# andrewcsmith/soundsym

Measured on NVIDIA B200. Metric: dtw_cell_updates_per_s, higher is better.
Workload: dtype f16 (packed-half DP scan on f16 tensor-core costs; winners refined in f64)

## Files before the change

soundsym_b200/csrc/dtw_h2.cu:

```cuda
#include <algorithm>
#include <atomic>
#include <type_traits>

#include "match.cuh"
#include "tc_common.cuh"

namespace ss {

int dtw_rescore_finalize(ss_dict* d, ss_queries* q, int k, int kp, uint32_t nslots, const uint32_t* d_slot_qid, double eps,
                         const float* d_max_na, const float* d_max_nb, const float* d_slot_max_na, int bound_mode, uint8_t* d_uncert_flag,
                         uint32_t* d_out_idx, double* d_out_dist);

int dtw_second_chance(ss_dict* d, ss_queries* q, int k, int kp, uint32_t nslots, const uint32_t* d_slot_qid, const unsigned long long* d_partial,
                      uint32_t nlists, const unsigned long long* d_thr, double eps, const float* d_max_na, const float* d_max_nb,
                      const float* d_slot_max_na, int bound_mode, uint8_t* d_uncert_flag, uint32_t* d_out_idx, double* d_out_dist);

constexpr int kH2Slots = 2;
constexpr int kH2SlotCols = 64;
constexpr int kH2DpWarps = 4 * kH2Slots;
constexpr int kH2DpThreads = kH2DpWarps * 32;
constexpr int kH2Threads = (kH2DpWarps + 1) * 32;
constexpr int kH2DescInt4 = 4;
constexpr int kH2In = 1, kH2Out = 2;
constexpr int kH2ARing = 32;
constexpr int kH2MaxLong = 2048;
constexpr int kH2Pipes = 2;
constexpr int kH2PDpWarps = kH2Pipes * kH2DpWarps;
constexpr int kH2PDpThreads = kH2PDpWarps * 32;
constexpr int kH2PThreads = (kH2PDpWarps + 4) * 32;
constexpr int kH2PRegsDp = 112, kH2PRegsProd = 32;
static_assert(kH2PDpThreads * kH2PRegsDp + 128 * kH2PRegsProd == kH2PThreads * 96, "setmaxnreg budget must match the launch pool");

struct H2Params {
    const unsigned char* a_blocks;
    const uint64_t* group_off;
    const uint32_t* group_len;
    const uint32_t* slot_len;
    uint32_t ngroups;
    const unsigned char* tiles;
    const int4* desc;
    const uint32_t* slice_tile;
    uint32_t nslices, slice_begin;
    unsigned long long* partial;
    uint32_t max_len;
    float inv_s;
    unsigned long long* thr;
    float* dbg;
    uint32_t dbg_nseg;
    __half2* bnd;
    uint32_t bnd_rows;
    float eta;
    unsigned long long* timeline;
};
__device__ __forceinline__ unsigned long long h2_now() {
    unsigned long long t;
    asm volatile("mov.u64 %0, %%globaltimer;" : "=l"(t));
    return t;
}

template <int N>
__device__ __forceinline__ void h2_ld(uint32_t taddr, __half2* v);
template <>
__device__ __forceinline__ void h2_ld<4>(uint32_t taddr, __half2* v) {
    uint32_t r[4];
    asm volatile("tcgen05.ld.sync.aligned.32x32b.x4.pack::16b.b32 {%0, %1, %2, %3}, [%4];\n" : "=r"(r[0]), "=r"(r[1]), "=r"(r[2]), "=r"(r[3]) : "r"(taddr));
#pragma unroll
    for (int i = 0; i < 4; i++) v[i] = *reinterpret_cast<__half2*>(&r[i]);
}
template <>
__device__ __forceinline__ void h2_ld<8>(uint32_t taddr, __half2* v) {
    uint32_t r[8];
    asm volatile("tcgen05.ld.sync.aligned.32x32b.x8.pack::16b.b32 {%0, %1, %2, %3, %4, %5, %6, %7}, [%8];\n"
                 : "=r"(r[0]), "=r"(r[1]), "=r"(r[2]), "=r"(r[3]), "=r"(r[4]), "=r"(r[5]), "=r"(r[6]), "=r"(r[7])
                 : "r"(taddr));
#pragma unroll
    for (int i = 0; i < 8; i++) v[i] = *reinterpret_cast<__half2*>(&r[i]);
}
template <>
__device__ __forceinline__ void h2_ld<16>(uint32_t taddr, __half2* v) {
    uint32_t r[16];
    asm volatile(
        "tcgen05.ld.sync.aligned.32x32b.x16.pack::16b.b32 {%0, %1, %2, %3, %4, %5, %6, %7, %8, %9, %10, %11, %12, %13, %14, %15}, [%16];\n"
        : "=r"(r[0]), "=r"(r[1]), "=r"(r[2]), "=r"(r[3]), "=r"(r[4]), "=r"(r[5]), "=r"(r[6]), "=r"(r[7]), "=r"(r[8]), "=r"(r[9]), "=r"(r[10]),
          "=r"(r[11]), "=r"(r[12]), "=r"(r[13]), "=r"(r[14]), "=r"(r[15])
        : "r"(taddr));
#pragma unroll
    for (int i = 0; i < 16; i++) v[i] = *reinterpret_cast<__half2*>(&r[i]);
}
template <int NG>
__device__ __forceinline__ void h2_ld_row(uint32_t taddr, __half2 (&v)[4 * NG]) {
    constexpr int N = 4 * NG;
    int done = 0;
    if constexpr (N >= 32) {
        h2_ld<16>(taddr, v);
        h2_ld<16>(taddr + 32, v + 16);
        done = 32;
    } else if constexpr (N >= 16) {
        h2_ld<16>(taddr, v);
        done = 16;
    }
    if constexpr ((N & 8) != 0) {
        h2_ld<8>(taddr + 2 * done, v + done);
        done += 8;
    }
    if constexpr ((N & 4) != 0) h2_ld<4>(taddr + 2 * done, v + done);
}

__device__ __forceinline__ __half2 h2_min3(__half2 a, __half2 b, __half2 c) { return __hmin2(__hmin2(a, b), c); }
__device__ __forceinline__ __half2 h2_inf() {
    const uint32_t bits = 0x7C007C00u;
    return *reinterpret_cast<const __half2*>(&bits);
}
__device__ __forceinline__ __half2 h2_zero() {
    const uint32_t bits = 0u;
    return *reinterpret_cast<const __half2*>(&bits);
}
__device__ __forceinline__ __half2 h2_combine(__half2 a, __half2 b) {
    const uint32_t r = __byte_perm(*reinterpret_cast<uint32_t*>(&a), *reinterpret_cast<uint32_t*>(&b), 0x7610);
    return *reinterpret_cast<const __half2*>(&r);
}
__device__ __forceinline__ int h2_len_of(const int4& sc, int e) { return (int)((((e < 4) ? (uint32_t)sc.x : (uint32_t)sc.y) >> (8 * (e & 3))) & 0xFFu); }
__device__ __forceinline__ int h2_seg_of(const int4& sa, const int4& sb, int e) {
    return e == 0 ? sa.x : e == 1 ? sa.y : e == 2 ? sa.z : e == 3 ? sa.w : e == 4 ? sb.x : e == 5 ? sb.y : e == 6 ? sb.z : sb.w;
}
__device__ __forceinline__ uint32_t h2_selp(uint32_t a, uint32_t b, int pick_a) {
    uint32_t r;
    asm("{\n.reg .pred q;\nsetp.ne.s32 q, %3, 0;\nselp.b32 %0, %1, %2, q;\n}\n" : "=r"(r) : "r"(a), "r"(b), "r"(pick_a));
    return r;
}
__device__ __forceinline__ __half2 h2_pick4(const __half2* v, int r) {
    const uint32_t v0 = *reinterpret_cast<const uint32_t*>(&v[0]), v1 = *reinterpret_cast<const uint32_t*>(&v[1]);
    const uint32_t v2 = *reinterpret_cast<const uint32_t*>(&v[2]), v3 = *reinterpret_cast<const uint32_t*>(&v[3]);
    const uint32_t lo = h2_selp(v1, v0, r & 1), hi = h2_selp(v3, v2, r & 1);
    const uint32_t o = h2_selp(hi, lo, r & 2);
    return *reinterpret_cast<const __half2*>(&o);
}

template <int NG>
__device__ __forceinline__ void h2_band(const __half2 (&tm0)[4 * NG], const __half2 (&tm1)[4 * NG], __half2 (&d)[4 * NG], __half2 dinit, __half2 (&c0l)[4]) {
    __half2 left0 = h2_inf(), diag0 = dinit, left1 = h2_inf();
#pragma unroll
    for (int j = 0; j < 4 * NG; j++) {
        const __half2 up0 = d[j];
        const __half2 c0 = __hadd2(tm0[j], h2_min3(left0, up0, diag0));
        const __half2 c1 = __hadd2(tm1[j], h2_min3(left1, c0, left0));
        diag0 = up0;
        left0 = c0;
        left1 = c1;
        d[j] = c1;
        if (j >= 4 * (NG - 1)) c0l[j - 4 * (NG - 1)] = c0;
    }
}
template <int NG>
__device__ __forceinline__ void h2_band_io(const __half2 (&tm0)[4 * NG], const __half2 (&tm1)[4 * NG], __half2 (&d)[4 * NG], __half2 l0, __half2 dg0,
                                           __half2 l1, __half2 (&c0l)[4], __half2& o0, __half2& o1) {
    __half2 left0 = l0, diag0 = dg0, left1 = l1;
#pragma unroll
    for (int j = 0; j < 4 * NG; j++) {
        const __half2 up0 = d[j];
        const __half2 c0 = __hadd2(tm0[j], h2_min3(left0, up0, diag0));
        const __half2 c1 = __hadd2(tm1[j], h2_min3(left1, c0, left0));
        diag0 = up0;
        left0 = c0;
        left1 = c1;
        d[j] = c1;
        if (j >= 4 * (NG - 1)) c0l[j - 4 * (NG - 1)] = c0;
    }
    o0 = left0, o1 = left1;
}
template <int NG>
__device__ __forceinline__ void h2_band_row_io(const __half2 (&tm)[4 * NG], __half2 (&d)[4 * NG], __half2 l0, __half2 dg0, __half2& o0) {
    __half2 left = l0, diag = dg0;
#pragma unroll
    for (int j = 0; j < 4 * NG; j++) {
        const __half2 up = d[j];
        const __half2 cur = __hadd2(tm[j], h2_min3(left, up, diag));
        diag = up;
        left = cur;
        d[j] = cur;
    }
    o0 = left;
}
template <int NG>
__device__ __forceinline__ void h2_band_row(const __half2 (&tm)[4 * NG], __half2 (&d)[4 * NG], __half2 dinit) {
    __half2 left = h2_inf(), diag = dinit;
#pragma unroll
    for (int j = 0; j < 4 * NG; j++) {
        const __half2 up = d[j];
        const __half2 cur = __hadd2(tm[j], h2_min3(left, up, diag));
        diag = up;
        left = cur;
        d[j] = cur;
    }
}

template <int NG, int J0, int J1>
__device__ __forceinline__ void h2_band_cols(const __half2* tm0, const __half2* tm1, __half2 (&d)[4 * NG], __half2& left0, __half2& diag0,
                                             __half2& left1, __half2 (&c0l)[4]) {
#pragma unroll
    for (int j = J0; j < J1; j++) {
        const __half2 up0 = d[j];
        const __half2 c0 = __hadd2(tm0[j - J0], h2_min3(left0, up0, diag0));
        const __half2 c1 = __hadd2(tm1[j - J0], h2_min3(left1, c0, left0));
        diag0 = up0;
        left0 = c0;
        left1 = c1;
        d[j] = c1;
        if (j >= 4 * (NG - 1)) c0l[j - 4 * (NG - 1)] = c0;
    }
}

struct H2PipeCursor {
    uint32_t par, full, taddr;
    __device__ __forceinline__ void wait() const {
        mb_wait_addr(full, par);
        tc_fence_after();
    }
    __device__ __forceinline__ void release() {
        tc_fence_before();
        mb_arrive_elect(full + 16);
        par ^= 1u;
    }
};

template <int NB, int NG, class Cur>
__device__ __forceinline__ void h2_step2(Cur& cur, __half2 (&d)[NB][4 * NG], __half2 dinit, __half2 (&c0l)[NB][4]) {
    constexpr int kBandCols = kH2SlotCols / NB;
    cur.wait();
    const uint32_t taddr = cur.taddr;
    if constexpr (std::is_same<Cur, H2PipeCursor>::value && NB == 1) {
        static_assert(NG >= 5, "NB = 1 tiles have 5..8 column groups");
        __half2 left0 = h2_inf(), diag0 = dinit, left1 = h2_inf();
        {
            __half2 a0[16], a1[16];
            h2_ld_row<4>(taddr, a0);
            h2_ld_row<4>(taddr + kTcN, a1);
            tc_wait_ld();
            h2_band_cols<NG, 0, 16>(a0, a1, d[0], left0, diag0, left1, c0l[0]);
        }
        __half2 b0[4 * (NG - 4)], b1[4 * (NG - 4)];
        h2_ld_row<NG - 4>(taddr + 32, b0);
        h2_ld_row<NG - 4>(taddr + kTcN + 32, b1);
        tc_wait_ld();
        cur.release();
        h2_band_cols<NG, 16, 4 * NG>(b0, b1, d[0], left0, diag0, left1, c0l[0]);
    } else if constexpr (std::is_same<Cur, H2PipeCursor>::value) {
        constexpr int H = NB / 2;
        {
            __half2 tm0[H][4 * NG], tm1[H][4 * NG];
#pragma unroll
            for (int b = 0; b < H; b++) {
                h2_ld_row<NG>(taddr + b * kBandCols, tm0[b]);
                h2_ld_row<NG>(taddr + kTcN + b * kBandCols, tm1[b]);
            }
            tc_wait_ld();
#pragma unroll
            for (int b = 0; b < H; b++) h2_band<NG>(tm0[b], tm1[b], d[b], dinit, c0l[b]);
        }
        __half2 tm0[H][4 * NG], tm1[H][4 * NG];
#pragma unroll
        for (int b = 0; b < H; b++) {
            h2_ld_row<NG>(taddr + (H + b) * kBandCols, tm0[b]);
            h2_ld_row<NG>(taddr + kTcN + (H + b) * kBandCols, tm1[b]);
        }
        tc_wait_ld();
        cur.release();
#pragma unroll
        for (int b = 0; b < H; b++) h2_band<NG>(tm0[b], tm1[b], d[H + b], dinit, c0l[H + b]);
    } else {
        __half2 tm0[NB][4 * NG], tm1[NB][4 * NG];
#pragma unroll
        for (int b = 0; b < NB; b++) {
            h2_ld_row<NG>(taddr + b * kBandCols, tm0[b]);
            h2_ld_row<NG>(taddr + kTcN + b * kBandCols, tm1[b]);
        }
        tc_wait_ld();
        cur.release();
#pragma unroll
        for (int b = 0; b < NB; b++) h2_band<NG>(tm0[b], tm1[b], d[b], dinit, c0l[b]);
    }
}

template <int NB, int NG, class Cur>
__device__ __forceinline__ void h2_tile(uint32_t L, uint32_t lmin, uint32_t Lm, const int4& sc, Cur& cur, __half2 (&res)[NB]) {
    __half2 d[NB][4 * NG];
#pragma unroll
    for (int b = 0; b < NB; b++) {
#pragma unroll
        for (int j = 0; j < 4 * NG; j++) d[b][j] = h2_inf();
        res[b] = h2_inf();
    }
    __half2 dinit = h2_zero();
    const uint32_t nfull = L >> 1;
    const uint32_t ncap = min((lmin - 1) >> 1, nfull);
    uint32_t st = 0;
    if constexpr (std::is_same<Cur, H2PipeCursor>::value) {
#pragma unroll 1
        for (; st < ncap; st++) {
            __half2 c0l[NB][4];
            h2_step2<NB, NG>(cur, d, dinit, c0l);
            dinit = h2_inf();
        }
    } else {
        if (st < ncap && cur.buf) {
            __half2 c0l[NB][4];
            h2_step2<NB, NG>(cur, d, dinit, c0l);
            dinit = h2_inf();
            st++;
        }
        if (st + 2 <= ncap) {
            const uint32_t full0 = cur.full, taddr0 = cur.taddr;
            uint32_t par = cur.par;
#pragma unroll 1
            for (; st + 2 <= ncap; st += 2) {
                __half2 c0l[NB][4];
                TcCursor c0 = {0u, par, full0, taddr0, cur.full_sum, cur.taddr_sum};
                h2_step2<NB, NG>(c0, d, dinit, c0l);
                TcCursor c1 = {1u, par, full0 + 8u, taddr0 + (uint32_t)kTcBufCols, cur.full_sum, cur.taddr_sum};
                h2_step2<NB, NG>(c1, d, h2_inf(), c0l);
                dinit = h2_inf();
                par ^= 1u;
            }
            cur.par = par;
        }
        if (st < ncap) {
            __half2 c0l[NB][4];
            h2_step2<NB, NG>(cur, d, dinit, c0l);
            dinit = h2_inf();
            st++;
        }
    }
#pragma unroll 1
    for (; st < nfull; st++) {
        __half2 c0l[NB][4];
        h2_step2<NB, NG>(cur, d, dinit, c0l);
        dinit = h2_inf();
        const bool end0 = 2 * st + 1 == Lm, end1 = 2 * st + 2 == Lm;
#pragma unroll
        for (int b = 0; b < NB; b++) {
            const int ra = (h2_len_of(sc, 2 * b) - 1) & 3, rb = (h2_len_of(sc, 2 * b + 1) - 1) & 3;
            const __half2 e0 = h2_combine(h2_pick4(c0l[b], ra), h2_pick4(c0l[b], rb));
            const __half2 e1 = h2_combine(h2_pick4(&d[b][4 * (NG - 1)], ra), h2_pick4(&d[b][4 * (NG - 1)], rb));
            res[b] = end0 ? e0 : (end1 ? e1 : res[b]);
        }
    }
    if (L & 1) {
        constexpr int kBandCols = kH2SlotCols / NB;
        cur.wait();
        __half2 tm0[NB][4 * NG];
#pragma unroll
        for (int b = 0; b < NB; b++) h2_ld_row<NG>(cur.taddr + b * kBandCols, tm0[b]);
        tc_wait_ld();
        cur.release();
#pragma unroll
        for (int b = 0; b < NB; b++) {
            h2_band_row<NG>(tm0[b], d[b], dinit);
            const int ra = (h2_len_of(sc, 2 * b) - 1) & 3, rb = (h2_len_of(sc, 2 * b + 1) - 1) & 3;
            const __half2 e = h2_combine(h2_pick4(&d[b][4 * (NG - 1)], ra), h2_pick4(&d[b][4 * (NG - 1)], rb));
            res[b] = (L == Lm) ? e : res[b];
        }
    }
}

template <int NG, bool IN, bool OUT>
__device__ __forceinline__ void h2_tile_strip(uint32_t L, uint32_t lmin, uint32_t Lm, const int4& sc, TcCursor& cur, __half2* bnd, __half2& res) {
    constexpr uint32_t kStride = kH2DpThreads;
    __half2 d[4 * NG];
#pragma unroll
    for (int j = 0; j < 4 * NG; j++) d[j] = h2_inf();
    res = h2_inf();
    __half2 prev_b = IN ? h2_inf() : h2_zero();
    const uint32_t nfull = L >> 1;
    const uint32_t ncap = OUT ? nfull : min((lmin - 1) >> 1, nfull);
    const int ra = (h2_len_of(sc, 0) - 1) & 3, rb = (h2_len_of(sc, 1) - 1) & 3;
#pragma unroll 1
    for (uint32_t st = 0; st < nfull; st++) {
        __half2 b0 = h2_inf(), b1 = h2_inf();
        if (IN) b0 = bnd[(size_t)(2 * st) * kStride], b1 = bnd[(size_t)(2 * st + 1) * kStride];
        cur.wait();
        const uint32_t taddr = cur.taddr;
        __half2 tm0[4 * NG], tm1[4 * NG], c0l[4], o0, o1;
        h2_ld_row<NG>(taddr, tm0);
        h2_ld_row<NG>(taddr + kTcN, tm1);
        tc_wait_ld();
        cur.release();
        h2_band_io<NG>(tm0, tm1, d, b0, prev_b, b1, c0l, o0, o1);
        prev_b = IN ? b1 : h2_inf();
        if (OUT) {
            bnd[(size_t)(2 * st) * kStride] = o0;
            bnd[(size_t)(2 * st + 1) * kStride] = o1;
        } else if (st >= ncap) {
            const bool end0 = 2 * st + 1 == Lm, end1 = 2 * st + 2 == Lm;
            const __half2 e0 = h2_combine(h2_pick4(c0l, ra), h2_pick4(c0l, rb));
            const __half2 e1 = h2_combine(h2_pick4(&d[4 * (NG - 1)], ra), h2_pick4(&d[4 * (NG - 1)], rb));
            res = end0 ? e0 : (end1 ? e1 : res);
        }
    }
    if (L & 1) {
        __half2 b0 = h2_inf();
        if (IN) b0 = bnd[(size_t)(L - 1) * kStride];
        cur.wait();
        __half2 tm0[4 * NG], o0;
        h2_ld_row<NG>(cur.taddr, tm0);
        tc_wait_ld();
        cur.release();
        h2_band_row_io<NG>(tm0, d, b0, prev_b, o0);
        if (OUT) {
            bnd[(size_t)(L - 1) * kStride] = o0;
        } else {
            const __half2 e = h2_combine(h2_pick4(&d[4 * (NG - 1)], ra), h2_pick4(&d[4 * (NG - 1)], rb));
            res = (L == Lm) ? e : res;
        }
    }
}

template <int KP, int NB, bool DBG = false>
__global__ void __launch_bounds__(kH2Threads, 1) k_dtw_scan_h2(const H2Params p) {
    extern __shared__ unsigned char smem_raw[];
    unsigned char* smem = smem_raw + ((128u - (s32(smem_raw) & 127u)) & 127u);
    unsigned char* sA = smem;
    unsigned char* sB = smem + (size_t)p.max_len * kTcATileBytes;
    uint64_t* bars = reinterpret_cast<uint64_t*>(sB + kTcStages * kTcBTileBytes);
    uint64_t* a_full = bars;
    uint64_t* b_full = bars + 1;
    uint64_t* b_empty = b_full + kTcStages;
    uint64_t* t_full = bars + 10;
    uint64_t* t_empty = bars + 12;
    uint32_t* tmem_slot = reinterpret_cast<uint32_t*>(bars + 14);
    unsigned long long* topk = reinterpret_cast<unsigned long long*>(bars + 32);

    const int warp = threadIdx.x >> 5, lane = threadIdx.x & 31;
    uint32_t g, slice;
    if (blockIdx.x < p.ngroups) {
        g = blockIdx.x, slice = p.slice_begin;
    } else {
        const uint32_t r = blockIdx.x - p.ngroups;
        g = r / (p.nslices - 1), slice = p.slice_begin + 1 + r % (p.nslices - 1);
    }
    asm volatile("griddepcontrol.launch_dependents;" ::: "memory");
    const uint32_t glen = p.group_len[g];
    const uint32_t L = glen & 0xFFFFu, lmin = glen >> 16;
    const uint32_t t0 = p.slice_tile[slice], t1 = p.slice_tile[slice + 1];
    const uint32_t ntiles = t1 - t0;
    unsigned long long* tl = p.timeline ? p.timeline + ((size_t)(p.slice_begin * p.ngroups) + blockIdx.x) * 8 : nullptr;
    if (tl && threadIdx.x == 0) {
        unsigned smid;
        asm("mov.u32 %0, %%smid;" : "=r"(smid));
        tl[0] = h2_now(), tl[4] = smid | ((unsigned long long)NB << 16) | ((unsigned long long)g << 32), tl[7] = ((unsigned long long)L << 32) | ntiles;
    }

    if (threadIdx.x == 0) {
        mb_init(a_full, 1);
        for (int s = 0; s < kTcStages; s++) mb_init(&b_full[s], 1), mb_init(&b_empty[s], 1);
        for (int s = 0; s < 2; s++) mb_init(&t_full[s], 1), mb_init(&t_empty[s], kH2DpWarps);
        asm volatile("fence.mbarrier_init.release.cluster;" ::: "memory");
    }
    if (warp == kH2DpWarps) {
        asm volatile("tcgen05.alloc.cta_group::1.sync.aligned.shared::cta.b32 [%0], %1;" ::"r"(s32(tmem_slot)), "r"(512u) : "memory");
        asm volatile("tcgen05.relinquish_alloc_permit.cta_group::1.sync.aligned;" ::: "memory");
    }
    tc_fence_before();
    __syncthreads();
    tc_fence_after();
    const uint32_t tmem_base = *tmem_slot;
    if (tl && threadIdx.x == 0) tl[1] = h2_now(), tl[5] = clock64();
    if (warp == kH2DpWarps) {
        if (lane == 0 && ntiles) {
            const uint32_t bars_s = s32(bars), sA_s = s32(sA), sB_s = s32(sB);
// ... 23 lines not shown
                    tc_mma_f16(tm, adesc, bdesc, idesc);
                    if (row + 1 < L) tc_mma_f16(tm + kTcN, adesc + (kTcATileBytes >> 4), bdesc, idesc);
                    tcs_commit(t_full_s + 8 * buf);
                    adesc += 2 * (kTcATileBytes >> 4);
                }
                tcs_commit(b_empty_s + 8 * stage);
                if (n + kTcStages < ntiles) {
                    mbs_wait_sleep(b_empty_s + 8 * stage, sphase);
                    mbs_expect_tx(b_full_s + 8 * stage, kTcBTileBytes);
                    tmas_g2s(sB_s + stage * kTcBTileBytes, tile_src, kTcBTileBytes, b_full_s + 8 * stage);
                    tile_src += kTcBTileBytes;
                }
                if (++stage == (uint32_t)kTcStages) stage = 0, sphase ^= 1;
            }
        }
    } else {
        const int q = warp & 3, slot = warp >> 2;
        const int m = q * 32 + lane;
        unsigned long long* list = topk + threadIdx.x;
#pragma unroll
        for (int s = 0; s < KP; s++) list[s * kH2DpThreads] = 0xFFFFFFFFFFFFFFFFull;
        const unsigned long long thr0 = __ldcg(p.thr + g * kTcM + m);
        unsigned long long worst = thr0;
        int cnt = 0, wpos = 0;
        const uint32_t lane_addr = tmem_base + ((uint32_t)(q * 32) << 16) + slot * kH2SlotCols;
        const uint32_t Lm = p.slot_len[g * kTcM + m];
        TcCursor cur;
        cur.init(s32(t_full), lane_addr);
        const int4* dp = p.desc + ((size_t)t0 * kH2Slots + slot) * kH2DescInt4;
        int4 na = make_int4(0, 0, 0, 0), nb = na, nc = na;
        if (ntiles) na = __ldg(dp), nb = __ldg(dp + 1), nc = __ldg(dp + 2);
        for (uint32_t n = 0; n < ntiles; n++) {
            const int4 sa = na, sb = nb, sc = nc;
            dp += kH2Slots * kH2DescInt4;
            if (n + 1 < ntiles) na = __ldg(dp), nb = __ldg(dp + 1), nc = __ldg(dp + 2);
            const int ng = sc.z;
            __half2 res[NB];
            if constexpr (NB == 1) {
                switch (ng) {
                    case 5: h2_tile<1, 5>(L, lmin, Lm, sc, cur, res); break;
                    case 6: h2_tile<1, 6>(L, lmin, Lm, sc, cur, res); break;
                    case 7: h2_tile<1, 7>(L, lmin, Lm, sc, cur, res); break;
                    default: h2_tile<1, 8>(L, lmin, Lm, sc, cur, res); break;
                }
            } else if constexpr (NB == 2) {
                if (ng == 3) h2_tile<2, 3>(L, lmin, Lm, sc, cur, res);
                else h2_tile<2, 4>(L, lmin, Lm, sc, cur, res);
            } else {
                if (ng == 1) h2_tile<4, 1>(L, lmin, Lm, sc, cur, res);
                else h2_tile<4, 2>(L, lmin, Lm, sc, cur, res);
            }
            if (tl && threadIdx.x == 0 && n + 1 == (ntiles + 1) / 2) tl[6] = h2_now();
            if (Lm) {
#pragma unroll
                for (int b = 0; b < NB; b++) {
#pragma unroll
                    for (int hsel = 0; hsel < 2; hsel++) {
                        const int e = 2 * b + hsel;
                        const int seg = h2_seg_of(sa, sb, e);
                        if (seg >= 0) {
                            const float v = hsel ? __high2float(res[b]) : __low2float(res[b]);
                            const float dist = __fdividef(v * p.inv_s, (float)(Lm + (uint32_t)h2_len_of(sc, e)));
                            const unsigned long long key = ((unsigned long long)tc_f2ord(dist) << 32) | (uint32_t)seg;
                            if (key < worst && dist == dist) {
                                const bool full = cnt == KP;
                                list[(full ? wpos : cnt) * kH2DpThreads] = key;
                                cnt += full ? 0 : 1;
                                if (cnt == KP) {
                                    tc_list_max<KP, kH2DpThreads>(list, worst, wpos);
                                    worst = worst < thr0 ? worst : thr0;
                                }
                            }
                            if constexpr (DBG) p.dbg[(size_t)(g * kTcM + m) * p.dbg_nseg + seg] = dist;
                        }
                    }
                }
            }
        }
        tc_sort_list<KP, kH2DpThreads>(list, cnt);
        worst = list[(KP - 1) * kH2DpThreads];
        worst = worst < thr0 ? worst : thr0;
        asm volatile("bar.sync 1, %0;" ::"n"(kH2DpThreads) : "memory");
        if (tl && threadIdx.x == 0) tl[2] = h2_now(), tl[5] = clock64() - tl[5];
        if (slot == 0) {
            const unsigned long long* other = list + kTcM;
            for (int s = 0; s < KP; s++) {
                const unsigned long long key = other[s * kH2DpThreads];
                if (key >= worst) break;
                tc_insert_key<KP, kH2DpThreads>(list, worst, key);
                worst = worst < thr0 ? worst : thr0;
            }
            const unsigned long long kept_worst = list[(KP - 1) * kH2DpThreads];
            if (kept_worst != 0xFFFFFFFFFFFFFFFFull && kept_worst < thr0) atomicMin(p.thr + g * kTcM + m, kept_worst);
            unsigned long long* out = p.partial + ((size_t)slice * p.ngroups * kTcM + (size_t)g * kTcM + m) * KP;
#pragma unroll
            for (int s = 0; s < KP; s++) out[s] = list[s * kH2DpThreads];
        }
    }
    if constexpr (NB != 1) asm volatile("griddepcontrol.wait;" ::: "memory");
    tc_fence_before();
    __syncthreads();
    if (warp == kH2DpWarps) {
        tc_fence_after();
        asm volatile("tcgen05.dealloc.cta_group::1.sync.aligned.b32 %0, %1;" ::"r"(tmem_base), "r"(512u) : "memory");
    }
    if (tl && threadIdx.x == 0) tl[3] = h2_now();
}

// ... 54 lines not shown
            const uint32_t a_full_s = bars_s, b_full_s = bars_s + 8 + pipe * (16 * kTcStages), b_empty_s = b_full_s + 8 * kTcStages,
                           t_full_s = s32(t_full) + 8 * pipe, t_empty_s = t_full_s + 16;
            if (pipe == 0) {
                mbs_expect_tx(a_full_s, L * kTcATileBytes);
                tmas_g2s(sA_s, p.a_blocks + p.group_off[g], L * kTcATileBytes, a_full_s);
            }
            constexpr size_t kStride = (size_t)kH2Pipes * kTcBTileBytes;
            const unsigned char* tile_src = p.tiles + (size_t)(t0 + pipe) * kTcBTileBytes;
            for (uint32_t n = 0; n < ntp && n < (uint32_t)kTcStages; n++) {
                mbs_expect_tx(b_full_s + 8 * n, kTcBTileBytes);
                tmas_g2s(sB_s + n * kTcBTileBytes, tile_src + n * kStride, kTcBTileBytes, b_full_s + 8 * n);
            }
            tile_src += kTcStages * kStride;
            mbs_wait_sleep(a_full_s, 0);
            const uint32_t idesc = (0u << 4) | ((uint32_t)(kTcN >> 3) << 17) | ((uint32_t)(kTcM >> 4) << 24);
            const uint64_t adesc0 = tc_smem_desc_s<kTcM>(sA_s);
            const uint32_t tm = tmem_base + pipe * kTcBufCols;
            uint32_t cnt = 0, stage = 0, sphase = 0;
            for (uint32_t n = 0; n < ntp; n++) {
                mbs_wait_sleep(b_full_s + 8 * stage, sphase);
                const uint64_t bdesc = tc_smem_desc_s<kTcN>(sB_s + stage * kTcBTileBytes);
                uint64_t adesc = adesc0;
                for (uint32_t row = 0; row < L; row += 2, cnt++) {
                    if (cnt >= 1) mbs_wait_sleep(t_empty_s, (cnt - 1) & 1);
                    tc_fence_after();
                    tc_mma_f16(tm, adesc, bdesc, idesc);
                    if (row + 1 < L) tc_mma_f16(tm + kTcN, adesc + (kTcATileBytes >> 4), bdesc, idesc);
                    tcs_commit(t_full_s);
                    adesc += 2 * (kTcATileBytes >> 4);
                }
                tcs_commit(b_empty_s + 8 * stage);
                if (n + kTcStages < ntp) {
                    mbs_wait_sleep(b_empty_s + 8 * stage, sphase);
                    mbs_expect_tx(b_full_s + 8 * stage, kTcBTileBytes);
                    tmas_g2s(sB_s + stage * kTcBTileBytes, tile_src, kTcBTileBytes, b_full_s + 8 * stage);
                    tile_src += kStride;
                }
                if (++stage == (uint32_t)kTcStages) stage = 0, sphase ^= 1;
            }
        }
    } else {
        asm volatile("setmaxnreg.inc.sync.aligned.u32 %0;" ::"n"(kH2PRegsDp));
        const int q = warp & 3, slot = (warp >> 2) & 1, pipe = warp >> 3;
        const int m = q * 32 + lane;
        unsigned long long* list = topk + threadIdx.x;
#pragma unroll
        for (int s = 0; s < KP; s++) list[s * kH2PDpThreads] = 0xFFFFFFFFFFFFFFFFull;
        const unsigned long long thr0 = __ldcg(p.thr + g * kTcM + m);
        unsigned long long worst = thr0;
        int cnt = 0, wpos = 0;
        const uint32_t Lm = p.slot_len[g * kTcM + m];
        H2PipeCursor cur = {0u, s32(t_full + pipe), tmem_base + ((uint32_t)(q * 32) << 16) + (uint32_t)(pipe * kTcBufCols + slot * kH2SlotCols)};
        const uint32_t ntp = ntiles > (uint32_t)pipe ? (ntiles - pipe + 1) >> 1 : 0u;
        const int4* dp = p.desc + ((size_t)(t0 + pipe) * kH2Slots + slot) * kH2DescInt4;
        int4 na = make_int4(0, 0, 0, 0), nb = na, nc = na;
        if (ntp) na = __ldg(dp), nb = __ldg(dp + 1), nc = __ldg(dp + 2);
        for (uint32_t n = 0; n < ntp; n++) {
            const int4 sa = na, sb = nb, sc = nc;
            dp += kH2Pipes * kH2Slots * kH2DescInt4;
            if (n + 1 < ntp) na = __ldg(dp), nb = __ldg(dp + 1), nc = __ldg(dp + 2);
            const int ng = sc.z;
            __half2 res[NB];
            if constexpr (NB == 1) {
                switch (ng) {
                    case 5: h2_tile<1, 5>(L, lmin, Lm, sc, cur, res); break;
                    case 6: h2_tile<1, 6>(L, lmin, Lm, sc, cur, res); break;
                    case 7: h2_tile<1, 7>(L, lmin, Lm, sc, cur, res); break;
                    default: h2_tile<1, 8>(L, lmin, Lm, sc, cur, res); break;
                }
            } else if constexpr (NB == 2) {
                if (ng == 3) h2_tile<2, 3>(L, lmin, Lm, sc, cur, res);
                else h2_tile<2, 4>(L, lmin, Lm, sc, cur, res);
            } else {
                if (ng == 1) h2_tile<4, 1>(L, lmin, Lm, sc, cur, res);
                else h2_tile<4, 2>(L, lmin, Lm, sc, cur, res);
            }
            if (tl && threadIdx.x == 0 && n + 1 == (ntp + 1) / 2) tl[6] = h2_now();
            if (Lm) {
#pragma unroll
                for (int b = 0; b < NB; b++) {
#pragma unroll
                    for (int hsel = 0; hsel < 2; hsel++) {
                        const int e = 2 * b + hsel;
                        const int seg = h2_seg_of(sa, sb, e);
                        if (seg >= 0) {
                            const float v = hsel ? __high2float(res[b]) : __low2float(res[b]);
                            const float dist = __fdividef(v * p.inv_s, (float)(Lm + (uint32_t)h2_len_of(sc, e)));
                            const unsigned long long key = ((unsigned long long)tc_f2ord(dist) << 32) | (uint32_t)seg;
                            if (key < worst && dist == dist) {
                                const bool full = cnt == KP;
                                list[(full ? wpos : cnt) * kH2PDpThreads] = key;
                                cnt += full ? 0 : 1;
                                if (cnt == KP) {
                                    tc_list_max<KP, kH2PDpThreads>(list, worst, wpos);
                                    worst = worst < thr0 ? worst : thr0;
                                }
                            }
                            if constexpr (DBG) p.dbg[(size_t)(g * kTcM + m) * p.dbg_nseg + seg] = dist;
                        }
                    }
                }
            }
        }
        tc_sort_list<KP, kH2PDpThreads>(list, cnt);
        worst = list[(KP - 1) * kH2PDpThreads];
        worst = worst < thr0 ? worst : thr0;
        asm volatile("bar.sync 1, %0;" ::"n"(kH2PDpThreads) : "memory");
        if (tl && threadIdx.x == 0) tl[2] = h2_now(), tl[5] = clock64() - tl[5];
        if (threadIdx.x < kTcM) {
            for (int o = 1; o < kH2Pipes * kH2Slots; o++) {
                const unsigned long long* other = list + o * kTcM;
                for (int s = 0; s < KP; s++) {
                    const unsigned long long key = other[s * kH2PDpThreads];
                    if (key >= worst) break;
                    tc_insert_key<KP, kH2PDpThreads>(list, worst, key);
                    worst = worst < thr0 ? worst : thr0;
                }
            }
            const unsigned long long kept_worst = list[(KP - 1) * kH2PDpThreads];
            if (kept_worst != 0xFFFFFFFFFFFFFFFFull && kept_worst < thr0) atomicMin(p.thr + g * kTcM + m, kept_worst);
            unsigned long long* out = p.partial + ((size_t)slice * p.ngroups * kTcM + (size_t)g * kTcM + m) * KP;
#pragma unroll
            for (int s = 0; s < KP; s++) out[s] = list[s * kH2PDpThreads];
        }
    }
    if constexpr (NB != 1) asm volatile("griddepcontrol.wait;" ::: "memory");
    tc_fence_before();
    __syncthreads();
    if (warp == kH2PDpWarps) {
        tc_fence_after();
        asm volatile("tcgen05.dealloc.cta_group::1.sync.aligned.b32 %0, %1;" ::"r"(tmem_base), "r"(512u) : "memory");
    }
    if (tl && threadIdx.x == 0) tl[3] = h2_now();
}

template <int KP, int NB, bool DBG = false>
__global__ void __launch_bounds__(kH2Threads, 1) k_dtw_scan_h2_long(const H2Params p) {
// ... 345 lines not shown
    d->h2_bmax = d->tc_max_abs;
    {
        DevBuf<uint32_t> d_n;
        SS_CUDA(ctx, d_n.reserve(1));
        k_h2_nsmid<<<1, 1, 0, ctx->stream>>>(d_n.p);
        SS_LAUNCHED(ctx);
        SS_CUDA(ctx, cudaMemcpyAsync(&d->h2_nsmid, d_n.p, sizeof(uint32_t), cudaMemcpyDeviceToHost, ctx->stream));
        SS_CUDA(ctx, cudaStreamSynchronize(ctx->stream));
    }
    d->h2_ready = true;
    return SS_OK;
}

static void h2_cost_scale(ss_dict* d, const ss_queries* q) {
    float S = d->h2_s0;
    for (uint64_t l = 64; l < (uint64_t)d->max_len + q->max_len && S > 1.0f / 65536.f; l *= 2) S *= 0.5f;
    d->h2_s = S;
}

static int h2_queries_build(ss_dict* d, ss_queries* q) {
    ss_ctx* ctx = q->ctx;
    h2_cost_scale(d, q);
    if (q->h2_built && q->h2_dict_serial == d->tc_serial && q->h2_s_built == d->h2_s) return SS_OK;
    if (!q->tc_grouped) SS_TRY(dtw_tc_queries_group(q));
    SS_CUDA(ctx, q->d_h2_a.reserve(std::max<uint64_t>(q->tc_a_bytes, 16)));
    SS_CUDA(ctx, q->d_tc_slot_max_na.reserve(std::max<size_t>((size_t)q->tc_ngroups * kTcM, 1)));
    SS_CUDA(ctx, q->d_uncert_flag.reserve(std::max<size_t>(q->nq, 1)));
    SS_CUDA(ctx, q->d_tc_max_norm.reserve(1));
    SS_CUDA(ctx, cudaMemsetAsync(q->d_tc_max_norm.p, 0, sizeof(float), ctx->stream));
    if (q->tc_ngroups) {
        SS_CUDA(ctx, cudaMemsetAsync(q->d_tc_slot_max_na.p, 0, (size_t)q->tc_ngroups * kTcM * sizeof(float), ctx->stream));
        k_tc_query_tiles<<<dim3(q->tc_ngroups, q->max_len), kTcM, 0, ctx->stream>>>(q->d_mfcc.p, q->d_off.p, q->c, d->d_mu.p, q->d_tc_group_len.p,
                                                                 q->d_tc_group_off.p, q->d_tc_qid.p, d->tc_nb_scale, d->h2_s, q->d_h2_a.p,
                                                                 q->d_tc_max_norm.p, q->d_tc_slot_max_na.p);
        SS_LAUNCHED(ctx);
    }
    q->h2_built = true;
    q->h2_dict_serial = d->tc_serial;
    q->h2_s_built = d->h2_s;
    return SS_OK;
}

constexpr int kH2Kp = 8;

template <int KP, int NB, bool DBG, bool LONG>
static int h2_launch_kind(ss_ctx* ctx, H2Params p, uint32_t slice_begin, uint32_t nslices, size_t smem, bool dependent) {
    if (!nslices) return SS_OK;
    p.slice_begin = slice_begin;
    p.nslices = nslices;
    void (*kern)(H2Params);
    unsigned threads = kH2Threads;
    if constexpr (LONG) {
        kern = k_dtw_scan_h2_long<KP, NB, DBG>;
    } else if constexpr (KP == kH2Kp && NB != 4) {
        kern = k_dtw_scan_h2_2p<KP, NB, DBG>;
        threads = kH2PThreads;
        smem = (size_t)p.max_len * kTcATileBytes + kH2Pipes * kTcStages * kTcBTileBytes + 32 * 8 + (size_t)KP * kH2PDpThreads * 8 + 1024;
    } else {
        kern = k_dtw_scan_h2<KP, NB, DBG>;
    }
    SS_CUDA(ctx, cudaFuncSetAttribute(kern, cudaFuncAttributeMaxDynamicSharedMemorySize, (int)smem));
    cudaLaunchConfig_t cfg = {};
    cfg.gridDim = dim3(p.ngroups * nslices);
    cfg.blockDim = dim3(threads);
    cfg.dynamicSmemBytes = smem;
    cfg.stream = ctx->stream;
    cudaLaunchAttribute attr[1];
    attr[0].id = cudaLaunchAttributeProgrammaticStreamSerialization;
    attr[0].val.programmaticStreamSerializationAllowed = 1;
    cfg.attrs = attr;
    cfg.numAttrs = dependent ? 1 : 0;
    SS_CUDA(ctx, cudaLaunchKernelEx(&cfg, kern, p));
    SS_LAUNCHED(ctx);
    return SS_OK;
}

static double h2_eta(const ss_dict* d) { return (13.0 * (double)d->h2_bmax + 4.0) * 5.9604644775390625e-08  / (double)d->h2_s; }

struct H2Plan {
    H2Params p;
    uint32_t kind_begin[4];
    uint32_t nslots;
    size_t smem;
    bool use_long;
};
constexpr int kH2Waves = 16;

static int h2_plan(ss_dict* d, ss_queries* q, int kp, H2Plan* plan) {
    ss_ctx* ctx = d->ctx;
    const uint32_t nslots = q->tc_ngroups * kTcM;
    if (d->h2_slices.size() > 64 && !d->h2_slices.count(q->tc_ngroups)) {
        SS_CUDA(ctx, cudaStreamSynchronize(ctx->stream));
        d->h2_slices.clear();
    }
    std::unique_ptr<ss_dict::H2Slices>& sl = d->h2_slices[q->tc_ngroups];
    if (!sl) {
        sl.reset(new ss_dict::H2Slices());
        const uint32_t want = std::max<uint32_t>(1, std::min<uint32_t>(((uint32_t)ctx->sm_count * kH2Waves + q->tc_ngroups - 1) / q->tc_ngroups,
                                                                       std::max<uint32_t>((uint32_t)ctx->sm_count, d->h2_ntiles / 12)));
        std::vector<uint32_t> st;
        uint64_t total = 0;
        for (uint32_t f : d->h_h2_tile_cost) total += f;
        const uint64_t per0 = std::max<uint64_t>(1, (total + want - 1) / want);
        int last_kind = -1, nkinds = 0;
        for (int kind = 0; kind < 3; kind++)
            if (d->h2_first_tile[kind + 1] > d->h2_first_tile[kind]) last_kind = kind, nkinds++;
        if (nkinds < 2) last_kind = -1;
        for (int kind = 0; kind < 3; kind++) {
            sl->kind_slice[kind] = (uint32_t)st.size();
            const uint64_t per = kind == last_kind ? std::max<uint64_t>(1, per0 / 2) : per0;
            uint64_t acc = per;
            for (uint32_t t = d->h2_first_tile[kind]; t < d->h2_first_tile[kind + 1]; t++) {
                if (acc >= per && !d->h_h2_tile_cont[t]) st.push_back(t), acc = 0;
                acc += d->h_h2_tile_cost[t];
            }
        }
        sl->kind_slice[3] = (uint32_t)st.size();
        st.push_back(d->h2_ntiles);
        SS_TRY(upload(ctx, sl->d_slice_tile, st.data(), st.size()));
    }
    const uint32_t nslices = sl->kind_slice[3];
    SS_CUDA(ctx, d->d_tc_partial.reserve((size_t)nslices * nslots * kp));
    SS_CUDA(ctx, d->d_cand_idx.reserve((size_t)nslots * kp));
    SS_CUDA(ctx, d->d_cand_adist.reserve((size_t)nslots * kp));
    if (!d->ev_scan0) {
        SS_CUDA(ctx, cudaEventCreate(&d->ev_scan0));
        SS_CUDA(ctx, cudaEventCreate(&d->ev_scan1));
    }
    H2Params& p = plan->p;
    p.a_blocks = q->d_h2_a.p;
    p.group_off = q->d_tc_group_off.p;
    p.group_len = q->d_tc_group_len.p;
    p.slot_len = q->d_tc_slot_len.p;
    p.ngroups = q->tc_ngroups;
    p.tiles = reinterpret_cast<const unsigned char*>(d->d_h2_tiles.p);
    p.desc = d->d_h2_desc.p;
    p.slice_tile = sl->d_slice_tile.p;
    p.nslices = nslices;
    p.slice_begin = 0;
    p.partial = d->d_tc_partial.p;
    p.max_len = q->max_len;
    p.inv_s = 1.0f / d->h2_s;
    SS_CUDA(ctx, d->d_h2_thr.reserve(std::max<uint32_t>(nslots, 1)));
    SS_CUDA(ctx, cudaMemsetAsync(d->d_h2_thr.p, 0xFF, (size_t)nslots * sizeof(unsigned long long), ctx->stream));
    p.thr = d->d_h2_thr.p;
    p.dbg = nullptr;
    p.dbg_nseg = 0;
    for (int i = 0; i < 4; i++) plan->kind_begin[i] = sl->kind_slice[i];
    plan->nslots = nslots;
    plan->use_long = d->h2_has_strips || q->max_len > (uint32_t)kTcMaxLen;
    p.bnd = nullptr;
    p.bnd_rows = 0;
    p.eta = 0.f;
    p.timeline = nullptr;
    if (plan->use_long) {
        if (d->h2_has_strips) {
            p.bnd_rows = (q->max_len + 1) & ~1u;
            SS_CUDA(ctx, d->d_h2_bnd.reserve((size_t)d->h2_nsmid * p.bnd_rows * kH2DpThreads));
            p.bnd = d->d_h2_bnd.p;
        }
        p.eta = (float)h2_eta(d) * 1.0001f;
        plan->smem = (size_t)kH2ARing * kTcATileBytes + kTcStages * kTcBTileBytes + 32 * 8 + (size_t)kp * kH2DpThreads * 8 + 1024;
    } else {
        plan->smem = (size_t)q->max_len * kTcATileBytes + kTcStages * kTcBTileBytes + 32 * 8 + (size_t)kp * kH2DpThreads * 8 + 1024;
    }
    return SS_OK;
}

template <int KP, bool DBG, bool LONG>
static int h2_launch_kinds(ss_ctx* ctx, const H2Plan& plan) {
    bool dep = false;
    const uint32_t* kb = plan.kind_begin;
    SS_TRY((h2_launch_kind<KP, 1, DBG, LONG>(ctx, plan.p, kb[0], kb[1] - kb[0], plan.smem, dep)));
    dep = dep || kb[1] > kb[0];
    SS_TRY((h2_launch_kind<KP, 2, DBG, LONG>(ctx, plan.p, kb[1], kb[2] - kb[1], plan.smem, dep)));
    dep = dep || kb[2] > kb[1];
    SS_TRY((h2_launch_kind<KP, 4, DBG, LONG>(ctx, plan.p, kb[2], kb[3] - kb[2], plan.smem, dep)));
    return SS_OK;
}
template <int KP, bool DBG>
static int h2_launch_all(ss_ctx* ctx, const H2Plan& plan) {
    return plan.use_long ? h2_launch_kinds<KP, DBG, true>(ctx, plan) : h2_launch_kinds<KP, DBG, false>(ctx, plan);
}

bool dtw_h2_applies(const ss_dict* d, const ss_queries* q) {
    return d->h2_ready && q->max_len <= (uint32_t)kH2MaxLong && q->total_frames > 0;
}

int dtw_h2_match_dev(ss_dict* d, ss_queries* q, int k, bool wide, bool second_chance, bool timed, uint32_t* d_out_idx, double* d_out_dist) {
    ss_ctx* ctx = d->ctx;
    TraceTimer tt(ctx);
    SS_TRY(h2_queries_build(d, q));
    tt.lap("  h2: query A blocks");
    const int kp = wide || k > 2 ? 32 : kH2Kp;
    H2Plan plan;
// ... 67 lines not shown
```

Before: 10250 billion.

## Prune top-k inserts with half2 bound test and route NB=4 to two-pipe kernel

Adds an early per-band rejection: the current worst key is converted back to a raw-scale float limit, and if both packed half results exceed it (with an upward-rounded slack) the per-element distance/division and list-insert work is skipped. The end-of-sequence result pick is moved into the step so the c0 snapshot only happens in the capture loop, and selects use predicated selp. The NB=4 tile kind now also uses the two-pipe warp-specialized kernel, with segment ids loaded lazily from global only when needed to save registers. This trades extra per-tile bound arithmetic and a register-pressure/scheduling change for fewer insert operations and better overlap for NB=4 tiles.

```diff
diff --git a/soundsym_b200/csrc/dtw_h2.cu b/soundsym_b200/csrc/dtw_h2.cu
--- a/soundsym_b200/csrc/dtw_h2.cu
+++ b/soundsym_b200/csrc/dtw_h2.cu
@@ -44,6 +44,7 @@
     unsigned long long* partial;
     uint32_t max_len;
     float inv_s;
+    float s;
     unsigned long long* thr;
     float* dbg;
     uint32_t dbg_nseg;
@@ -128,6 +129,10 @@
     asm("{\n.reg .pred q;\nsetp.ne.s32 q, %3, 0;\nselp.b32 %0, %1, %2, q;\n}\n" : "=r"(r) : "r"(a), "r"(b), "r"(pick_a));
     return r;
 }
+__device__ __forceinline__ __half2 h2_sel(__half2 a, __half2 b, bool pick_a) {
+    const uint32_t o = h2_selp(*reinterpret_cast<const uint32_t*>(&a), *reinterpret_cast<const uint32_t*>(&b), pick_a ? 1 : 0);
+    return *reinterpret_cast<const __half2*>(&o);
+}
 __device__ __forceinline__ __half2 h2_pick4(const __half2* v, int r) {
     const uint32_t v0 = *reinterpret_cast<const uint32_t*>(&v[0]), v1 = *reinterpret_cast<const uint32_t*>(&v[1]);
     const uint32_t v2 = *reinterpret_cast<const uint32_t*>(&v[2]), v3 = *reinterpret_cast<const uint32_t*>(&v[3]);
@@ -223,27 +228,33 @@
     }
 };
 
-template <int NB, int NG, class Cur>
-__device__ __forceinline__ void h2_step2(Cur& cur, __half2 (&d)[NB][4 * NG], __half2 dinit, __half2 (&c0l)[NB][4]) {
+__device__ __forceinline__ __half2 h2_end_pick(const __half2* v, const int4& sc, int b) {
+    const int ra = (h2_len_of(sc, 2 * b) - 1) & 3, rb = (h2_len_of(sc, 2 * b + 1) - 1) & 3;
+    return h2_combine(h2_pick4(v, ra), h2_pick4(v, rb));
+}
+
+template <int NB, int NG, bool CAP, class Cur>
+__device__ __forceinline__ void h2_step2(Cur& cur, __half2 (&d)[NB][4 * NG], __half2 dinit, const int4& sc, __half2 (&e0)[NB]) {
     constexpr int kBandCols = kH2SlotCols / NB;
     cur.wait();
     const uint32_t taddr = cur.taddr;
     if constexpr (std::is_same<Cur, H2PipeCursor>::value && NB == 1) {
         static_assert(NG >= 5, "NB = 1 tiles have 5..8 column groups");
-        __half2 left0 = h2_inf(), diag0 = dinit, left1 = h2_inf();
+        __half2 left0 = h2_inf(), diag0 = dinit, left1 = h2_inf(), c0l[4];
         {
             __half2 a0[16], a1[16];
             h2_ld_row<4>(taddr, a0);
             h2_ld_row<4>(taddr + kTcN, a1);
             tc_wait_ld();
-            h2_band_cols<NG, 0, 16>(a0, a1, d[0], left0, diag0, left1, c0l[0]);
+            h2_band_cols<NG, 0, 16>(a0, a1, d[0], left0, diag0, left1, c0l);
         }
         __half2 b0[4 * (NG - 4)], b1[4 * (NG - 4)];
         h2_ld_row<NG - 4>(taddr + 32, b0);
         h2_ld_row<NG - 4>(taddr + kTcN + 32, b1);
         tc_wait_ld();
         cur.release();
-        h2_band_cols<NG, 16, 4 * NG>(b0, b1, d[0], left0, diag0, left1, c0l[0]);
+        h2_band_cols<NG, 16, 4 * NG>(b0, b1, d[0], left0, diag0, left1, c0l);
+        if constexpr (CAP) e0[0] = h2_end_pick(c0l, sc, 0);
     } else if constexpr (std::is_same<Cur, H2PipeCursor>::value) {
         constexpr int H = NB / 2;
         {
@@ -255,7 +266,11 @@
             }
             tc_wait_ld();
 #pragma unroll
-            for (int b = 0; b < H; b++) h2_band<NG>(tm0[b], tm1[b], d[b], dinit, c0l[b]);
+            for (int b = 0; b < H; b++) {
+                __half2 c0l[4];
+                h2_band<NG>(tm0[b], tm1[b], d[b], dinit, c0l);
+                if constexpr (CAP) e0[b] = h2_end_pick(c0l, sc, b);
+            }
         }
         __half2 tm0[H][4 * NG], tm1[H][4 * NG];
 #pragma unroll
@@ -266,7 +281,11 @@
         tc_wait_ld();
         cur.release();
 #pragma unroll
-        for (int b = 0; b < H; b++) h2_band<NG>(tm0[b], tm1[b], d[H + b], dinit, c0l[H + b]);
+        for (int b = 0; b < H; b++) {
+            __half2 c0l[4];
+            h2_band<NG>(tm0[b], tm1[b], d[H + b], dinit, c0l);
+            if constexpr (CAP) e0[H + b] = h2_end_pick(c0l, sc, H + b);
+        }
     } else {
         __half2 tm0[NB][4 * NG], tm1[NB][4 * NG];
 #pragma unroll
@@ -277,7 +296,11 @@
         tc_wait_ld();
         cur.release();
 #pragma unroll
-        for (int b = 0; b < NB; b++) h2_band<NG>(tm0[b], tm1[b], d[b], dinit, c0l[b]);
+        for (int b = 0; b < NB; b++) {
+            __half2 c0l[4];
+            h2_band<NG>(tm0[b], tm1[b], d[b], dinit, c0l);
+            if constexpr (CAP) e0[b] = h2_end_pick(c0l, sc, b);
+        }
     }
 }
 
@@ -294,17 +317,16 @@
     const uint32_t nfull = L >> 1;
     const uint32_t ncap = min((lmin - 1) >> 1, nfull);
     uint32_t st = 0;
+    __half2 e0[NB];
     if constexpr (std::is_same<Cur, H2PipeCursor>::value) {
 #pragma unroll 1
         for (; st < ncap; st++) {
-            __half2 c0l[NB][4];
-            h2_step2<NB, NG>(cur, d, dinit, c0l);
+            h2_step2<NB, NG, false>(cur, d, dinit, sc, e0);
             dinit = h2_inf();
         }
     } else {
         if (st < ncap && cur.buf) {
-            __half2 c0l[NB][4];
-            h2_step2<NB, NG>(cur, d, dinit, c0l);
+            h2_step2<NB, NG, false>(cur, d, dinit, sc, e0);
             dinit = h2_inf();
             st++;
         }
@@ -313,35 +335,30 @@
             uint32_t par = cur.par;
 #pragma unroll 1
             for (; st + 2 <= ncap; st += 2) {
-                __half2 c0l[NB][4];
                 TcCursor c0 = {0u, par, full0, taddr0, cur.full_sum, cur.taddr_sum};
-                h2_step2<NB, NG>(c0, d, dinit, c0l);
+                h2_step2<NB, NG, false>(c0, d, dinit, sc, e0);
                 TcCursor c1 = {1u, par, full0 + 8u, taddr0 + (uint32_t)kTcBufCols, cur.full_sum, cur.taddr_sum};
-                h2_step2<NB, NG>(c1, d, h2_inf(), c0l);
+                h2_step2<NB, NG, false>(c1, d, h2_inf(), sc, e0);
                 dinit = h2_inf();
                 par ^= 1u;
             }
             cur.par = par;
         }
         if (st < ncap) {
-            __half2 c0l[NB][4];
-            h2_step2<NB, NG>(cur, d, dinit, c0l);
+            h2_step2<NB, NG, false>(cur, d, dinit, sc, e0);
             dinit = h2_inf();
             st++;
         }
     }
 #pragma unroll 1
     for (; st < nfull; st++) {
-        __half2 c0l[NB][4];
-        h2_step2<NB, NG>(cur, d, dinit, c0l);
+        h2_step2<NB, NG, true>(cur, d, dinit, sc, e0);
         dinit = h2_inf();
         const bool end0 = 2 * st + 1 == Lm, end1 = 2 * st + 2 == Lm;
 #pragma unroll
         for (int b = 0; b < NB; b++) {
-            const int ra = (h2_len_of(sc, 2 * b) - 1) & 3, rb = (h2_len_of(sc, 2 * b + 1) - 1) & 3;
-            const __half2 e0 = h2_combine(h2_pick4(c0l[b], ra), h2_pick4(c0l[b], rb));
-            const __half2 e1 = h2_combine(h2_pick4(&d[b][4 * (NG - 1)], ra), h2_pick4(&d[b][4 * (NG - 1)], rb));
-            res[b] = end0 ? e0 : (end1 ? e1 : res[b]);
+            const __half2 e1 = h2_end_pick(&d[b][4 * (NG - 1)], sc, b);
+            res[b] = h2_sel(e0[b], h2_sel(e1, res[b], end1), end0);
         }
     }
     if (L & 1) {
@@ -355,9 +372,7 @@
 #pragma unroll
         for (int b = 0; b < NB; b++) {
             h2_band_row<NG>(tm0[b], d[b], dinit);
-            const int ra = (h2_len_of(sc, 2 * b) - 1) & 3, rb = (h2_len_of(sc, 2 * b + 1) - 1) & 3;
-            const __half2 e = h2_combine(h2_pick4(&d[b][4 * (NG - 1)], ra), h2_pick4(&d[b][4 * (NG - 1)], rb));
-            res[b] = (L == Lm) ? e : res[b];
+            res[b] = h2_sel(h2_end_pick(&d[b][4 * (NG - 1)], sc, b), res[b], L == Lm);
         }
     }
 }
@@ -414,6 +429,15 @@
     }
 }
 
+__device__ __forceinline__ float h2_key_float(unsigned long long key) {
+    const uint32_t o = (uint32_t)(key >> 32);
+    return o >= 0xFF800000u ? __int_as_float(0x7F800000) : __uint_as_float((o & 0x80000000u) ? (o & 0x7FFFFFFFu) : ~o);
+}
+__device__ __forceinline__ __half2 h2_raw_limits(float ws, uint32_t Lm, const int4& sc, int b) {
+    const float xa = ws * (float)(Lm + (uint32_t)h2_len_of(sc, 2 * b)), xb = ws * (float)(Lm + (uint32_t)h2_len_of(sc, 2 * b + 1));
+    return __halves2half2(__float2half_ru(fmaf(fabsf(xa), 0x1p-10f, xa)), __float2half_ru(fmaf(fabsf(xb), 0x1p-10f, xb)));
+}
+
 template <int KP, int NB, bool DBG = false>
 __global__ void __launch_bounds__(kH2Threads, 1) k_dtw_scan_h2(const H2Params p) {
     extern __shared__ unsigned char smem_raw[];
@@ -543,8 +567,12 @@
             }
             if (tl && threadIdx.x == 0 && n + 1 == (ntiles + 1) / 2) tl[6] = h2_now();
             if (Lm) {
+                const float ws = h2_key_float(worst) * p.s;
 #pragma unroll
                 for (int b = 0; b < NB; b++) {
+                    if constexpr (!DBG) {
+                        if (__hbgtu2(res[b], h2_raw_limits(ws, Lm, sc, b))) continue;
+                    }
 #pragma unroll
                     for (int hsel = 0; hsel < 2; hsel++) {
                         const int e = 2 * b + hsel;
@@ -705,13 +733,20 @@
         const uint32_t Lm = p.slot_len[g * kTcM + m];
         H2PipeCursor cur = {0u, s32(t_full + pipe), tmem_base + ((uint32_t)(q * 32) << 16) + (uint32_t)(pipe * kTcBufCols + slot * kH2SlotCols)};
         const uint32_t ntp = ntiles > (uint32_t)pipe ? (ntiles - pipe + 1) >> 1 : 0u;
+        constexpr bool kLazyIds = NB == 4;
+        constexpr uint32_t kDescStride = kH2Pipes * kH2Slots * kH2DescInt4;
         const int4* dp = p.desc + ((size_t)(t0 + pipe) * kH2Slots + slot) * kH2DescInt4;
         int4 na = make_int4(0, 0, 0, 0), nb = na, nc = na;
-        if (ntp) na = __ldg(dp), nb = __ldg(dp + 1), nc = __ldg(dp + 2);
-        for (uint32_t n = 0; n < ntp; n++) {
+        if (ntp) {
+            nc = __ldg(dp + 2);
+            if constexpr (!kLazyIds) na = __ldg(dp), nb = __ldg(dp + 1);
+        }
+        for (uint32_t n = 0; n < ntp; n++, dp += kDescStride) {
             const int4 sa = na, sb = nb, sc = nc;
-            dp += kH2Pipes * kH2Slots * kH2DescInt4;
-            if (n + 1 < ntp) na = __ldg(dp), nb = __ldg(dp + 1), nc = __ldg(dp + 2);
+            if (n + 1 < ntp) {
+                nc = __ldg(dp + kDescStride + 2);
+                if constexpr (!kLazyIds) na = __ldg(dp + kDescStride), nb = __ldg(dp + kDescStride + 1);
+            }
             const int ng = sc.z;
             __half2 res[NB];
             if constexpr (NB == 1) {
@@ -730,12 +765,16 @@
             }
             if (tl && threadIdx.x == 0 && n + 1 == (ntp + 1) / 2) tl[6] = h2_now();
             if (Lm) {
+                const float ws = h2_key_float(worst) * p.s;
 #pragma unroll
                 for (int b = 0; b < NB; b++) {
+                    if constexpr (!DBG) {
+                        if (__hbgtu2(res[b], h2_raw_limits(ws, Lm, sc, b))) continue;
+                    }
 #pragma unroll
                     for (int hsel = 0; hsel < 2; hsel++) {
                         const int e = 2 * b + hsel;
-                        const int seg = h2_seg_of(sa, sb, e);
+                        const int seg = kLazyIds ? __ldg(reinterpret_cast<const int*>(dp) + e) : h2_seg_of(sa, sb, e);
                         if (seg >= 0) {
                             const float v = hsel ? __high2float(res[b]) : __low2float(res[b]);
                             const float dist = __fdividef(v * p.inv_s, (float)(Lm + (uint32_t)h2_len_of(sc, e)));
@@ -1187,7 +1226,7 @@
     unsigned threads = kH2Threads;
     if constexpr (LONG) {
         kern = k_dtw_scan_h2_long<KP, NB, DBG>;
-    } else if constexpr (KP == kH2Kp && NB != 4) {
+    } else if constexpr (KP == kH2Kp) {
         kern = k_dtw_scan_h2_2p<KP, NB, DBG>;
         threads = kH2PThreads;
         smem = (size_t)p.max_len * kTcATileBytes + kH2Pipes * kTcStages * kTcBTileBytes + 32 * 8 + (size_t)KP * kH2PDpThreads * 8 + 1024;
@@ -1276,6 +1315,7 @@
     p.partial = d->d_tc_partial.p;
     p.max_len = q->max_len;
     p.inv_s = 1.0f / d->h2_s;
+    p.s = d->h2_s;
     SS_CUDA(ctx, d->d_h2_thr.reserve(std::max<uint32_t>(nslots, 1)));
     SS_CUDA(ctx, cudaMemsetAsync(d->d_h2_thr.p, 0xFF, (size_t)nslots * sizeof(unsigned long long), ctx->stream));
     p.thr = d->d_h2_thr.p;
```

New measurement: 10260 billion, median of 6. No clear change (+0.1%).
